# aidalee123/Vision-SR

Measured on NVIDIA B200. Metric: candidate_fits_per_sec, higher is better.
Workload: dtype f64

## Files before the change

vision-sr_b200/csrc/vsr_api.cu:

```cuda
#include <algorithm>
#include <cstdarg>
#include <cstdio>
#include <cstdlib>
#include <cstring>
#include <string>
#include <mutex>
#include <vector>

#include "../../include/vsr.h"
#define VSR_API_TU 1
#include "vsr_launch.h"

namespace {

constexpr int kWidths[] = {0, 1, 2, 3, 4, 5, 6, 7, 8, 12, 16};
constexpr int kNumWidths = sizeof(kWidths) / sizeof(kWidths[0]);

int pick_width(int k) {
  for (int w : kWidths)
    if (w >= k) return w;
  return -1;
}

std::string g_create_error;
// ... 46 lines not shown
  }
};

struct PointSlot {
  const void* X = nullptr;
  const void* y = nullptr;
  int64_t n = 0, ldx = 0;
  int n_vars = 0;
  DevBuf ownX, ownY;
};

}

constexpr int kPoolStreams = 32;
constexpr int kHandleStride = 8;
constexpr int kMaxGroups = 16;
struct StreamPool {
  std::mutex mu;
  std::vector<cudaStream_t> streams;
  int next_base = 0;
};
StreamPool& pool_of(int device) {
  static StreamPool pools[64];
  return pools[device & 63];
}

struct vsr_handle {
  int device = 0;
  int stream_base = 0;
  int num_sms = 148;
  std::string err;
  PointSlot pts[2];
  DevBuf d_insns, d_insn_off, d_imms, d_imm_off, d_k;
  std::vector<int32_t> h_k, h_ninsn, h_nimm, h_nvars;
  std::vector<uint32_t> h_varmask;
  std::vector<cudaStream_t> side_streams;
  cudaEvent_t ev_fork = nullptr;
  std::vector<cudaEvent_t> ev_join;
  int n_programs = 0;
  DevBuf d_lists;
  DevBuf d_partial;
  DevBuf d_stage;
  DevBuf d_queue;
  DevBuf d_handover;
  PinnedBuf h_lists;
  int64_t launches = 0;
  int hook[4] = {0, 0, 0, 0};
  int tile_smem_kb = 200;
  int64_t tile_min_points = 500000;
  int steal_span = 3;
  int latency_k = 0;
  bool queue_by_candidate = false;
  bool handover = true;
  int hold_passes = 500;
  bool profiling = false;
  long long* phase_cycles = nullptr;
  struct Span {
    cudaEvent_t a, b;
    int kind, n;
  };
  std::vector<Span> spans;
  std::vector<cudaEvent_t> event_pool;
};

namespace {

// ... 374 lines not shown
      if (e == cudaSuccess) sp.streams.push_back(s2);
    }
    h->stream_base = sp.next_base;
    sp.next_base = (sp.next_base + kHandleStride) % kPoolStreams;
    for (int i = 0; i < kHandleStride; ++i) h->side_streams.push_back(sp.streams[(h->stream_base + i) % kPoolStreams]);
    for (int i = 0; i < kMaxGroups && e == cudaSuccess; ++i) {
      cudaEvent_t e2;
      e = cudaEventCreateWithFlags(&e2, cudaEventDisableTiming);
      if (e == cudaSuccess) h->ev_join.push_back(e2);
    }
  }
  if (e == cudaSuccess) e = cudaEventCreateWithFlags(&h->ev_fork, cudaEventDisableTiming);
  if (e != cudaSuccess) {
    fail(nullptr, VSR_ECUDA, "allocating the handle's scratch: %s", cudaGetErrorString(e));
    vsr_destroy(h);
    return VSR_ECUDA;
  }
  *out = h;
  return VSR_OK;
}

void vsr_destroy(vsr_handle* h) {
  if (!h) return;
  cudaSetDevice(h->device);
  for (auto& s : h->pts) {
    s.ownX.release();
    s.ownY.release();
  }
  h->d_insns.release();
  h->d_insn_off.release();
  h->d_imms.release();
  h->d_imm_off.release();
  h->d_k.release();
  h->d_lists.release();
  h->d_partial.release();
  h->d_stage.release();
  h->d_queue.release();
  h->d_handover.release();
  h->h_lists.release();
  for (auto e2 : h->ev_join) cudaEventDestroy(e2);
  if (h->ev_fork) cudaEventDestroy(h->ev_fork);
  for (auto& sp : h->spans) {
    if (sp.kind == 0) h->event_pool.push_back(sp.a);
    h->event_pool.push_back(sp.b);
  }
  for (auto e : h->event_pool) cudaEventDestroy(e);
  delete h;
}

const char* vsr_last_error(const vsr_handle* h) { return h ? h->err.c_str() : g_create_error.c_str(); }

int64_t vsr_launch_count(const vsr_handle* h) { return h ? h->launches : 0; }

int vsr_set_phase_buffer(vsr_handle* h, void* dev_i64_nslots_by_8) {
  if (!h) return VSR_EINVAL;
  h->phase_cycles = (long long*)dev_i64_nslots_by_8;
  return VSR_OK;
}

int vsr_set_geometry(vsr_handle* h, int32_t cluster, int32_t threads, int32_t seats, int32_t opt_warps) {
  if (!h) return VSR_EINVAL;
  h->hook[0] = cluster;
  h->hook[1] = threads;
  h->hook[2] = seats;
  h->hook[3] = opt_warps;
  return VSR_OK;
// ... 83 lines not shown
    const int ni = insn_off[c + 1] - insn_off[c];
    const int nm = imm_off[c + 1] - imm_off[c];
    if (ni < 1 || ni > VSR_MAX_INSNS || nm < 0 || nm > VSR_MAX_IMMS || k[c] < 0 || k[c] > VSR_MAX_CONSTS)
      return fail(h, VSR_ELIMIT, "program %d: %d insns, %d literals, %d constants", c, ni, nm, k[c]);
    if (VSR_OP(insns[insn_off[c + 1] - 1]) != VSR_END)
      return fail(h, VSR_EINVAL, "program %d does not end in END", c);
    int sp = 0;
    unsigned var_mask = 0;
    for (int i = insn_off[c]; i < insn_off[c + 1]; ++i) {
      const unsigned op = VSR_OP(insns[i]), src = VSR_SRC(insns[i]), idx = VSR_IDX(insns[i]);
      if (op >= VSR_OP_COUNT) return fail(h, VSR_EINVAL, "program %d: bad opcode %u", c, op);
      if (op == VSR_PUSH && ++sp > VSR_MAX_STACK) return fail(h, VSR_ELIMIT, "program %d: stack too deep", c);
      if (op >= VSR_LOAD && op <= VSR_RPOW && op != VSR_PUSH) {
        if (src == VSR_SRC_STACK) {
          if (--sp < 0) return fail(h, VSR_EINVAL, "program %d: stack underflow", c);
        } else if (src == VSR_SRC_VAR) {
          if (idx >= VSR_MAX_VARS) return fail(h, VSR_EINVAL, "program %d: variable %u", c, idx);
          var_mask |= 1u << idx;
        } else if (src == VSR_SRC_CONST) {
          if ((int)idx >= k[c]) return fail(h, VSR_EINVAL, "program %d: constant %u of %d", c, idx, k[c]);
        } else if (src == VSR_SRC_IMM) {
          if ((int)idx >= nm) return fail(h, VSR_EINVAL, "program %d: literal %u of %d", c, idx, nm);
        } else {
          return fail(h, VSR_EINVAL, "program %d: bad operand source %u", c, src);
        }
      }
    }
    h->h_ninsn[c] = ni;
    h->h_nimm[c] = nm;
    h->h_nvars[c] = __builtin_popcount(var_mask);
    h->h_varmask[c] = var_mask;
  }
  const size_t nins = insn_off[n_programs], nimm = std::max(1, imm_off[n_programs]);
  VSR_CUDA(h, h->d_insns.reserve(nins * sizeof(uint64_t)));
  VSR_CUDA(h, h->d_insn_off.reserve((n_programs + 1) * sizeof(int32_t)));
  VSR_CUDA(h, h->d_imms.reserve(nimm * sizeof(double)));
  VSR_CUDA(h, h->d_imm_off.reserve((n_programs + 1) * sizeof(int32_t)));
  VSR_CUDA(h, h->d_k.reserve(n_programs * sizeof(int32_t)));
  VSR_CUDA(h, cudaMemcpyAsync(h->d_insns.p, insns, nins * sizeof(uint64_t), cudaMemcpyHostToDevice, st));
  VSR_CUDA(h, cudaMemcpyAsync(h->d_insn_off.p, insn_off, (n_programs + 1) * sizeof(int32_t), cudaMemcpyHostToDevice, st));
  if (imm_off[n_programs] > 0)
    VSR_CUDA(h, cudaMemcpyAsync(h->d_imms.p, imms, imm_off[n_programs] * sizeof(double), cudaMemcpyHostToDevice, st));
  VSR_CUDA(h, cudaMemcpyAsync(h->d_imm_off.p, imm_off, (n_programs + 1) * sizeof(int32_t), cudaMemcpyHostToDevice, st));
  VSR_CUDA(h, cudaMemcpyAsync(h->d_k.p, k, n_programs * sizeof(int32_t), cudaMemcpyHostToDevice, st));
  h->n_programs = n_programs;
  return VSR_OK;
}

int vsr_eval(vsr_handle* h, const int32_t* prog_idx, const int32_t* const_row, int32_t n_pairs,
             const double* consts, int32_t kstride, int32_t dtype, double* out_loss,
             double* out_grad, void* stream) {
  int rc = check_ready(h, dtype);
  if (rc) return rc;
  if (!prog_idx || n_pairs <= 0 || !out_loss || kstride < 0 || (!consts && kstride > 0))
    return fail(h, VSR_EINVAL, "bad eval arguments");
  cudaStream_t st = (cudaStream_t)stream;
  VSR_CUDA(h, cudaSetDevice(h->device));
  std::vector<Group> groups(kNumWidths + 1);
  for (int i = 0; i < kNumWidths; ++i) groups[i].K = kWidths[i];
  Group& toowide = groups[kNumWidths];
  for (int p = 0; p < n_pairs; ++p) {
    const int c = prog_idx[p];
    if (c < 0 || c >= h->n_programs) return fail(h, VSR_EINVAL, "pair %d: program %d out of range", p, c);
    const int k = h->h_k[c];
    if (k > kstride) return fail(h, VSR_EINVAL, "pair %d: %d constants > kstride %d", p, k, kstride);
    if ((rc = check_vars(h, c, dtype))) return rc;
    int gi = 0;
    if (out_grad) {
      const int w = pick_width(k);
      if (w < 0) {
        toowide.prog.push_back(p);
        gi = 0;
      } else {
        gi = (int)(std::find(kWidths, kWidths + kNumWidths, w) - kWidths);
      }
    }
    Group& g = groups[gi];
// ... 340 lines not shown
  const bool tma_ok = ((uintptr_t)ps.X % 16 == 0) && ((uintptr_t)ps.y % 16 == 0) && ((ps.ldx * elem) % 16 == 0);
  cudaEvent_t ev_a = nullptr, ev_b = nullptr, ev_c = nullptr;
  if (h->profiling) {
    ev_a = take_event(h);
    ev_b = take_event(h);
    ev_c = take_event(h);
    VSR_CUDA(h, cudaEventRecord(ev_a, st));
  }
  VSR_CUDA(h, h->d_queue.reserve(groups.size() * sizeof(int32_t)));
  VSR_CUDA(h, cudaMemsetAsync(h->d_queue.p, 0, groups.size() * sizeof(int32_t), st));
  std::vector<size_t> ho_off(groups.size() + 1, 0);
  std::vector<int> ho_slot_d(groups.size(), 0);
  if (h->handover) {
    for (size_t gi = 0; gi < groups.size(); ++gi) {
      ho_slot_d[gi] = (vsr::kHandoverHead + vsr::kFitStateDoubles + vsr::fit_workspace_doubles(std::max(1, groups[gi].kmax)) + 1) & ~1;
      ho_off[gi + 1] = ho_off[gi] + 16 + (size_t)vsr::kHandoverSlots * ho_slot_d[gi] * sizeof(double);
    }
    VSR_CUDA(h, h->d_handover.reserve(ho_off.back()));
    VSR_CUDA(h, cudaMemsetAsync(h->d_handover.p, 0, ho_off.back(), st));
  }
  const int hook_cluster = h->hook[0], hook_threads = h->hook[1], hook_seats = h->hook[2], hook_reserved = h->hook[3];

  const size_t n_side = groups.size() > 1 ? groups.size() - 1 : 0;
  if (n_side > h->ev_join.size()) return fail(h, VSR_EINVAL, "%zu launch groups: too many", n_side + 1);
  if (n_side && !h->ev_fork) VSR_CUDA(h, cudaEventCreateWithFlags(&h->ev_fork, cudaEventDisableTiming));
  if (n_side) VSR_CUDA(h, cudaEventRecord(h->ev_fork, st));
  for (size_t gi = 0; gi < groups.size(); ++gi) {
    Group& g = groups[gi];
    const int n = (int)g.prog.size();
    cudaStream_t gs = gi == 0 ? st : h->side_streams[(gi - 1) % h->side_streams.size()];
    if (gi > 0) VSR_CUDA(h, cudaStreamWaitEvent(gs, h->ev_fork, 0));
    vsr::FitArgs a;
    a.pt = table_of(h);
    a.pts = points_of(ps);
    a.run_prog = dl;
    a.run_slot = dl + n_listed;
    a.n_queues = 0;
    for (size_t gj = gi; gj < groups.size() && a.n_queues < vsr::kMaxQueues; ++gj) {
      if (gj > gi && (groups[gj].grad_mode != g.grad_mode || groups[gj].K == 0 || g.K - groups[gj].K > h->steal_span ||
                      gj != gi + (size_t)a.n_queues))
        break;
      a.q_begin[a.n_queues] = g_begin[gj];
      a.q_end[a.n_queues] = g_begin[gj + 1];
      ++a.n_queues;
    }
    for (int q = a.n_queues; q < vsr::kMaxQueues; ++q) a.q_begin[q] = a.q_end[q] = 0;
    a.kstride = kstride;
    a.x0 = x0;
    a.out_consts = out_consts;
    a.out_lastx = out_lastx;
    a.out_loss = out_loss;
    a.out_info = out_info;
    a.O.gtol = opts->gtol;
    a.O.c1 = opts->c1;
    a.O.c2 = opts->c2;
    a.O.xrtol = opts->xrtol;
    a.O.fd_eps = opts->fd_eps;
    a.O.penalty = opts->penalty;
    a.O.loss_scale = opts->loss_scale;
    a.O.stop_time = opts->stop_time;
    a.O.maxiter_per_k = opts->maxiter_per_k;
    a.O.grad_mode = g.grad_mode;
    const int P = points_per_thread(g.K);
    int cap = opts->eval_dtype == VSR_F64 ? fit_threads_cap<double>(g.K) : fit_threads_cap<float>(g.K);
    if (hook_threads > 0) cap = std::min(cap, std::max(32, hook_threads & ~31));
    if (h->latency_k > 0 && g.K >= h->latency_k && hook_threads <= 0) cap = std::min(cap, 320);
// ... 100 lines not shown
```

vision-sr_b200/csrc/vsr_interp.h:

```cpp
#ifndef VSR_INTERP_H_
#define VSR_INTERP_H_

#include "vsr_isa.h"

#if defined(__CUDACC__)
#define VSR_HD __host__ __device__ __forceinline__
#define VSR_MATH __host__ __device__ __noinline__ inline
#else
#include <cmath>
#define VSR_HD inline
#define VSR_MATH inline
#endif

namespace vsr {

#define VSR_M1(Q, name, fd, ff)                 \
  Q double name(double x) { return fd(x); }     \
  Q float name(float x) { return ff(x); }
VSR_M1(VSR_HD, m_sqrt, ::sqrt, ::sqrtf)
VSR_M1(VSR_HD, m_abs, ::fabs, ::fabsf)
VSR_M1(VSR_MATH, m_exp, ::exp, ::expf)
VSR_M1(VSR_MATH, m_log, ::log, ::logf)
VSR_M1(VSR_MATH, m_sin, ::sin, ::sinf)
VSR_M1(VSR_MATH, m_cos, ::cos, ::cosf)
VSR_M1(VSR_MATH, m_tan, ::tan, ::tanf)
VSR_M1(VSR_MATH, m_asin, ::asin, ::asinf)
VSR_M1(VSR_MATH, m_acos, ::acos, ::acosf)
VSR_M1(VSR_MATH, m_atan, ::atan, ::atanf)
VSR_M1(VSR_MATH, m_sinh, ::sinh, ::sinhf)
VSR_M1(VSR_MATH, m_cosh, ::cosh, ::coshf)
VSR_M1(VSR_MATH, m_tanh, ::tanh, ::tanhf)
#undef VSR_M1
VSR_MATH double m_pow(double a, double b) { return ::pow(a, b); }
VSR_MATH float m_pow(float a, float b) { return ::powf(a, b); }
// ... 24 lines not shown
#endif
}
template <typename T>
VSR_HD T m_sign(T x) {
  return x > T(0) ? T(1) : (x < T(0) ? T(-1) : (x == T(0) ? T(0) : x));
}
template <typename T>
VSR_HD T m_powi(T x, int n) {
  T r = T(1);
  T b = x;
  while (n > 0) {
    if (n & 1) r *= b;
    n >>= 1;
    if (n) b *= b;
  }
  return r;
}
template <typename T>
VSR_HD T m_scale(T d, T fp) {
  return d == T(0) ? T(0) : d * fp;
}

template <typename T, int K>
struct Dual {
  T v;
  T d[K > 0 ? K : 1];
};

template <typename T, int K, int P>
struct Stack {
  T s[VSR_MAX_STACK][P][K + 1];
};

template <int OP, typename T, int K>
VSR_HD void unary_apply(Dual<T, K>& x, unsigned am, int n) {
  const T a = x.v;
  const bool live = (K > 0) && am != 0u;
  T f = a, fp = T(1);
  bool guard = false;
  switch (OP) {
    case VSR_NEG:
      f = -a;
      fp = T(-1);
      break;
    case VSR_ABS:
      f = m_abs(a);
      fp = m_sign(a);
      break;
    case VSR_SIGN:
      f = m_sign(a);
      fp = T(0);
      break;
    case VSR_INV:
      f = T(1) / a;
      fp = -f * f;
      break;
    case VSR_SQRT:
      f = m_sqrt(a);
      fp = T(0.5) / f;
      guard = true;
      break;
    case VSR_EXP:
      f = m_exp(a);
      fp = f;
      break;
    case VSR_LOG:
      f = m_log(a);
      fp = T(1) / a;
      break;
    case VSR_SIN:
      if (live) {
        m_sincos(a, &f, &fp);
      } else {
        f = m_sin(a);
      }
      break;
    case VSR_COS:
      if (live) {
        T s;
        m_sincos(a, &s, &f);
        fp = -s;
      } else {
        f = m_cos(a);
      }
      break;
    case VSR_TAN:
      f = m_tan(a);
      fp = T(1) + f * f;
      break;
    case VSR_ASIN:
      f = m_asin(a);
      if (live) fp = T(1) / m_sqrt(T(1) - a * a);
      guard = true;
      break;
    case VSR_ACOS:
      f = m_acos(a);
      if (live) fp = T(-1) / m_sqrt(T(1) - a * a);
      guard = true;
      break;
    case VSR_ATAN:
      f = m_atan(a);
      fp = T(1) / (T(1) + a * a);
      break;
    case VSR_SINH:
      f = m_sinh(a);
      if (live) fp = m_cosh(a);
      break;
    case VSR_COSH:
      f = m_cosh(a);
      if (live) fp = m_sinh(a);
      break;
    case VSR_TANH:
      f = m_tanh(a);
      fp = T(1) - f * f;
      break;
    case VSR_POWI: {
      const int m = n < 0 ? -n : n;
      const T pw = m_powi(a, m - 1);
      const T full = pw * a;
      if (n > 0) {
        f = full;
        fp = T(n) * pw;
      } else {
        f = T(1) / full;
        fp = T(n) * f / a;
      }
      break;
    }
    default:
      break;
  }
  x.v = f;
  if (K > 0) {
    if (guard) {
#pragma unroll
      for (int i = 0; i < K; ++i) x.d[i] = m_scale(x.d[i], fp);
    } else {
#pragma unroll
      for (int i = 0; i < K; ++i) x.d[i] *= fp;
    }
  }
}

#define VSR_H_BINOP(op) ((op) == VSR_LOAD ? 0 : (op)-VSR_ADD + 1)
#define VSR_H_BIN(op, src) (2 + ((VSR_H_BINOP(op)) << 2) + (src))
#define VSR_H_UN(op) (38 + (op)-VSR_NEG)
#define VSR_H_CFOP(op) ((op) == VSR_LOAD ? 0 : (op) == VSR_ADD ? 1 : (op) == VSR_SUB ? 2 : 3)
#define VSR_H_CF(op, j) (55 + VSR_H_CFOP(op) * VSR_MAX_DUAL + (j))
#define VSR_H_END 0
#define VSR_H_PUSH 1
#define VSR_H_COUNT 119
#define VSR_HANDLER(w) ((unsigned)((w)&0xff))

VSR_HD vsr_insn_t predecode(vsr_insn_t w) {
  const unsigned op = VSR_OP(w);
  unsigned h;
  if (op == VSR_END)
    h = VSR_H_END;
  else if (op == VSR_PUSH)
    h = VSR_H_PUSH;
  else if ((op == VSR_LOAD || op == VSR_ADD || op == VSR_SUB || op == VSR_MUL) &&
           (VSR_SRC(w) & 3u) == VSR_SRC_CONST && VSR_IDX(w) < VSR_MAX_DUAL &&
           (op == VSR_LOAD || !((VSR_AMASK(w) >> VSR_IDX(w)) & 1u)))
    h = VSR_H_CF(op, VSR_IDX(w));
  else if (op <= VSR_RPOW)
    h = VSR_H_BIN(op, VSR_SRC(w) & 3u);
  else
    h = VSR_H_UN(op);
  return (w & ~(vsr_insn_t)0xff) | (vsr_insn_t)h;
}

template <int OP, int SRC, typename T, int K, int P, typename XSrc>
VSR_HD void binary_apply(Dual<T, K> (&acc)[P], Stack<T, K, P>& stk, int& sp, unsigned idx,
                         unsigned am, unsigned bm, const double* __restrict__ imm,
                         const T* __restrict__ cst, const XSrc& xs) {
  if (SRC == VSR_SRC_STACK) --sp;
  T ub = T(0);
  if (SRC == VSR_SRC_CONST) ub = cst[idx];
  if (SRC == VSR_SRC_IMM) ub = (T)imm[idx];
  const unsigned lm = am | bm;
#pragma unroll
  for (int p = 0; p < P; ++p) {
    T bv;
    if (SRC == VSR_SRC_STACK)
      bv = stk.s[sp][p][0];
    else if (SRC == VSR_SRC_VAR)
      bv = xs.col(idx, p);
    else
      bv = ub;
    Dual<T, K>& x = acc[p];
#define VSR_TB(i)                                                                   \
  (SRC == VSR_SRC_STACK ? (((bm >> (i)) & 1u) ? stk.s[sp][p][(i) + 1] : T(0))      \
                        : (SRC == VSR_SRC_CONST ? ((i) == (int)idx ? T(1) : T(0)) : T(0)))
    switch (OP) {
      case VSR_LOAD:
        x.v = bv;
#pragma unroll
        for (int i = 0; i < K; ++i) x.d[i] = VSR_TB(i);
        break;
      case VSR_ADD:
        x.v += bv;
        if (SRC == VSR_SRC_STACK) {
#pragma unroll
          for (int i = 0; i < K; ++i)
            if ((bm >> i) & 1u) x.d[i] += stk.s[sp][p][i + 1];
        } else if (SRC == VSR_SRC_CONST) {
#pragma unroll
          for (int i = 0; i < K; ++i) x.d[i] += VSR_TB(i);
        }
        break;
      case VSR_SUB:
        x.v -= bv;
        if (SRC == VSR_SRC_STACK) {
#pragma unroll
          for (int i = 0; i < K; ++i)
            if ((bm >> i) & 1u) x.d[i] -= stk.s[sp][p][i + 1];
        } else if (SRC == VSR_SRC_CONST) {
#pragma unroll
          for (int i = 0; i < K; ++i) x.d[i] -= VSR_TB(i);
        }
        break;
      case VSR_RSUB:
        x.v = bv - x.v;
#pragma unroll
        for (int i = 0; i < K; ++i) x.d[i] = VSR_TB(i) - x.d[i];
        break;
      case VSR_MUL: {
        const T a = x.v;
        x.v = a * bv;
        if (SRC == VSR_SRC_STACK) {
#pragma unroll
          for (int i = 0; i < K; ++i)
            if ((lm >> i) & 1u) x.d[i] = x.d[i] * bv + a * VSR_TB(i);
        } else if (SRC == VSR_SRC_CONST) {
#pragma unroll
          for (int i = 0; i < K; ++i) x.d[i] = x.d[i] * bv + (i == (int)idx ? a : T(0));
        } else {
#pragma unroll
          for (int i = 0; i < K; ++i) x.d[i] *= bv;
        }
        break;
      }
      case VSR_DIV: {
        const T inv = T(1) / bv;
        const T q = x.v / bv;
        if (SRC == VSR_SRC_STACK) {
#pragma unroll
          for (int i = 0; i < K; ++i)
            if ((lm >> i) & 1u) x.d[i] = (x.d[i] - q * VSR_TB(i)) * inv;
        } else if (SRC == VSR_SRC_CONST) {
#pragma unroll
          for (int i = 0; i < K; ++i) x.d[i] = (x.d[i] - (i == (int)idx ? q : T(0))) * inv;
        } else {
#pragma unroll
          for (int i = 0; i < K; ++i) x.d[i] *= inv;
        }
        x.v = q;
        break;
      }
      case VSR_RDIV: {
        const T a = x.v;
        const T inv = T(1) / a;
        const T q = bv / a;
        if (SRC == VSR_SRC_STACK) {
#pragma unroll
          for (int i = 0; i < K; ++i)
            if ((lm >> i) & 1u) x.d[i] = (VSR_TB(i) - q * x.d[i]) * inv;
        } else if (SRC == VSR_SRC_CONST) {
#pragma unroll
          for (int i = 0; i < K; ++i) x.d[i] = ((i == (int)idx ? T(1) : T(0)) - q * x.d[i]) * inv;
        } else {
          const T cf = -q * inv;
#pragma unroll
          for (int i = 0; i < K; ++i) x.d[i] *= cf;
        }
        x.v = q;
        break;
      }
      case VSR_POW: {
        const T a = x.v;
        T lna = T(0);
        const T f = (K == 0) ? m_pow(a, bv) : m_pow_log(a, bv, lna);
        if (K > 0 && lm) {
          const T fa = am ? (a != T(0) ? bv * (f / a) : bv * m_pow(a, bv - T(1))) : T(0);
          T fb = T(0);
          if (bm) fb = (a == T(0) && f == T(0)) ? T(0) : f * lna;
#pragma unroll
          for (int i = 0; i < K; ++i)
            if ((lm >> i) & 1u) x.d[i] = m_scale(x.d[i], fa) + m_scale((T)VSR_TB(i), fb);
        }
        x.v = f;
        break;
      }
      case VSR_RPOW: {
        const T a = x.v;
        T lnb = T(0);
        const T f = (K == 0) ? m_pow(bv, a) : m_pow_log(bv, a, lnb);
        if (K > 0 && lm) {
          T fa = T(0);
          if (am) fa = (bv == T(0) && f == T(0)) ? T(0) : f * lnb;
          const T fb = bm ? (bv != T(0) ? a * (f / bv) : a * m_pow(bv, a - T(1))) : T(0);
#pragma unroll
          for (int i = 0; i < K; ++i)
            if ((lm >> i) & 1u) x.d[i] = m_scale(x.d[i], fa) + m_scale((T)VSR_TB(i), fb);
        }
        x.v = f;
        break;
      }
      default:
        break;
    }
#undef VSR_TB
  }
}

template <int OP, int J, typename T, int K, int P>
VSR_HD void const_fresh_apply(Dual<T, K> (&acc)[P], const T* __restrict__ cst) {
  constexpr int JJ = (K > 0 && J < K) ? J : 0;
  const T c = cst[J];
#pragma unroll
  for (int p = 0; p < P; ++p) {
    Dual<T, K>& x = acc[p];
    const T a = x.v;
    switch (OP) {
      case VSR_LOAD:
        x.v = c;
#pragma unroll
        for (int i = 0; i < K; ++i) x.d[i] = T(0);
        if (K > 0) x.d[JJ] = T(1);
        break;
      case VSR_ADD:
        x.v = a + c;
        if (K > 0) x.d[JJ] = T(1);
        break;
      case VSR_SUB:
        x.v = a - c;
        if (K > 0) x.d[JJ] = T(-1);
        break;
      case VSR_MUL:
        x.v = a * c;
#pragma unroll
        for (int i = 0; i < K; ++i)
          if (i != JJ) x.d[i] *= c;
        if (K > 0) x.d[JJ] = a;
        break;
      default:
        break;
    }
  }
}

template <typename T, int K, int P, typename XSrc>
VSR_HD void eval_points(const vsr_insn_t* __restrict__ prog, const double* __restrict__ imm,
                        const T* __restrict__ cst, const XSrc& xs, Dual<T, K> (&acc)[P],
                        Stack<T, K, P>& stk) {
  int sp = 0;
#pragma unroll
  for (int p = 0; p < P; ++p) {
    acc[p].v = T(0);
#pragma unroll
    for (int i = 0; i < (K > 0 ? K : 1); ++i) acc[p].d[i] = T(0);
  }
  vsr_insn_t w = prog[0];
  for (int pc = 1;; ++pc) {
    const unsigned hid = VSR_HANDLER(w);
    const unsigned idx = VSR_IDX(w);
    const unsigned am = VSR_AMASK(w);
    const unsigned bm = VSR_BMASK(w);
    w = prog[pc];
    switch (hid) {
      case VSR_H_END:
        return;
      case VSR_H_PUSH:
#pragma unroll
        for (int p = 0; p < P; ++p) {
          stk.s[sp][p][0] = acc[p].v;
#pragma unroll
          for (int i = 0; i < K; ++i)
            if ((am >> i) & 1u) stk.s[sp][p][i + 1] = acc[p].d[i];
        }
        ++sp;
        break;
#define VSR_BCASE(OPC)                                                                          \
  case VSR_H_BIN(OPC, VSR_SRC_STACK):                                                           \
    binary_apply<OPC, VSR_SRC_STACK, T, K, P>(acc, stk, sp, idx, am, bm, imm, cst, xs);         \
    break;                                                                                      \
  case VSR_H_BIN(OPC, VSR_SRC_VAR):                                                             \
    binary_apply<OPC, VSR_SRC_VAR, T, K, P>(acc, stk, sp, idx, am, bm, imm, cst, xs);           \
    break;                                                                                      \
  case VSR_H_BIN(OPC, VSR_SRC_CONST):                                                           \
    binary_apply<OPC, VSR_SRC_CONST, T, K, P>(acc, stk, sp, idx, am, bm, imm, cst, xs);         \
    break;                                                                                      \
  case VSR_H_BIN(OPC, VSR_SRC_IMM):                                                             \
    binary_apply<OPC, VSR_SRC_IMM, T, K, P>(acc, stk, sp, idx, am, bm, imm, cst, xs);           \
    break;
        VSR_BCASE(VSR_LOAD)
        VSR_BCASE(VSR_ADD)
        VSR_BCASE(VSR_SUB)
        VSR_BCASE(VSR_RSUB)
        VSR_BCASE(VSR_MUL)
        VSR_BCASE(VSR_DIV)
        VSR_BCASE(VSR_RDIV)
        VSR_BCASE(VSR_POW)
        VSR_BCASE(VSR_RPOW)
#undef VSR_BCASE
#define VSR_CFCASE1(OPC, J)                                              \
  case VSR_H_CF(OPC, J):                                                 \
    if (J < K || K == 0) const_fresh_apply<OPC, J, T, K, P>(acc, cst);   \
    break;
#define VSR_CFCASE(OPC)                                                                          \
  VSR_CFCASE1(OPC, 0) VSR_CFCASE1(OPC, 1) VSR_CFCASE1(OPC, 2) VSR_CFCASE1(OPC, 3)                \
  VSR_CFCASE1(OPC, 4) VSR_CFCASE1(OPC, 5) VSR_CFCASE1(OPC, 6) VSR_CFCASE1(OPC, 7)                \
  VSR_CFCASE1(OPC, 8) VSR_CFCASE1(OPC, 9) VSR_CFCASE1(OPC, 10) VSR_CFCASE1(OPC, 11)              \
  VSR_CFCASE1(OPC, 12) VSR_CFCASE1(OPC, 13) VSR_CFCASE1(OPC, 14) VSR_CFCASE1(OPC, 15)
        VSR_CFCASE(VSR_LOAD)
        VSR_CFCASE(VSR_ADD)
        VSR_CFCASE(VSR_SUB)
        VSR_CFCASE(VSR_MUL)
#undef VSR_CFCASE
#undef VSR_CFCASE1
#define VSR_UCASE(OPC)                                                  \
  case VSR_H_UN(OPC):                                                   \
    _Pragma("unroll") for (int p = 0; p < P; ++p)                       \
        unary_apply<OPC, T, K>(acc[p], am, (int)(int16_t)idx);          \
    break;
        VSR_UCASE(VSR_NEG)
        VSR_UCASE(VSR_ABS)
        VSR_UCASE(VSR_SIGN)
        VSR_UCASE(VSR_INV)
        VSR_UCASE(VSR_SQRT)
        VSR_UCASE(VSR_EXP)
        VSR_UCASE(VSR_LOG)
        VSR_UCASE(VSR_SIN)
        VSR_UCASE(VSR_COS)
        VSR_UCASE(VSR_TAN)
        VSR_UCASE(VSR_ASIN)
        VSR_UCASE(VSR_ACOS)
        VSR_UCASE(VSR_ATAN)
        VSR_UCASE(VSR_SINH)
        VSR_UCASE(VSR_COSH)
        VSR_UCASE(VSR_TANH)
        VSR_UCASE(VSR_POWI)
#undef VSR_UCASE
      default:
#if defined(__CUDA_ARCH__)
        __builtin_unreachable();
#else
        break;
#endif
    }
  }
}

}

#endif
```

vision-sr_b200/csrc/vsr_kernels.cuh:

```cuda
#ifndef VSR_KERNELS_CUH_
#define VSR_KERNELS_CUH_

#include <cooperative_groups.h>
#include <cuda_runtime.h>
#include <stdint.h>

#include "vsr_bfgs.h"
#include "vsr_interp.h"
#include "vsr_isa.h"

namespace vsr {

struct ProgramTable {
  const vsr_insn_t* insns;
  const int32_t* insn_off;
  const double* imms;
  const int32_t* imm_off;
  const int32_t* k;
};

struct Points {
  const void* X;
  const void* y;
  int64_t n;
  int64_t ldx;
};

constexpr int kHandoverSlots = 64;
constexpr unsigned long long kHandoverWaitNs = 300000ull;
constexpr int kHandoverHead = 4;
struct Handover {
  int32_t requests;
  int32_t offers;
  int32_t live;
  int32_t pad;
  double slots[1];
};

constexpr int kMaxSeats = 8;
constexpr int kMaxQueues = 4;

struct FitArgs {
  ProgramTable pt;
  Points pts;
  const int32_t* run_prog;
  const int32_t* run_slot;
  int32_t n_queues;
  int32_t q_begin[kMaxQueues], q_end[kMaxQueues];
  int32_t kstride;
  const double* x0;
  double* out_consts;
  double* out_lastx;
  double* out_loss;
  int32_t* out_info;
  int32_t resident;
  int32_t tma_ok;
  int32_t slice_stride;
  int32_t seats;
  int32_t reserved;
  int32_t seat_d, off_cred, off_ctrl, off_insn;
  int32_t kmax, max_insn, max_imm;
  int32_t n_cols;
  int32_t col_of_var[VSR_MAX_VARS];
  int32_t hold_passes;
  Handover* handover;
  int32_t handover_slot_d;
  int32_t* queue;
  long long* phase_cycles;
  FitOpts O;
};

struct EvalArgs {
  ProgramTable pt;
  Points pts;
  const int32_t* pair_prog;
  const int32_t* pair_row;
// ... 360 lines not shown

struct SeatCtrl {
  int prog;
  int k;
  int n_insn;
  int age;
};

struct SeatBook {
  int slot;
  int prog;
  int k;
  int pad;
  unsigned long long t0;
  double rf;
  long long t_logic, t_seated, n_pass, t_take, t_step, t_pub, ns_seated;
};

template <typename T>
__device__ __forceinline__ void publish_request(const FitArgs& a, int cs, int lane, int prog, int k, bool fresh, int age,
                                                const double* xe, uint32_t ctrl_addr, uint32_t req_bar_addr) {
  int i0 = 0, ni = 0, m0 = 0, nm = 0;
  if (prog >= 0 && fresh) {
    i0 = a.pt.insn_off[prog];
    ni = a.pt.insn_off[prog + 1] - i0;
    m0 = a.pt.imm_off[prog];
    nm = a.pt.imm_off[prog + 1] - m0;
  }
  const uint32_t bytes = 16u + (prog >= 0 ? (uint32_t)k * (uint32_t)sizeof(T) : 0u) +
                         (fresh && prog >= 0 ? (uint32_t)(nm + ni + 1) * 8u : 0u);
  for (int r = lane; r < cs; r += 32) mbar_expect_tx_cluster(mapa_u32(req_bar_addr, r), bytes);
  const uint32_t cst_addr = ctrl_addr + 8u * kSeatCtrlDoubles;
  {
    const int n_items = 2 + (prog >= 0 ? k : 0);
    const int sh = __ffs(cs) - 1;
    for (int idx = lane; idx < (n_items << sh); idx += 32) {
      const int r = idx & (cs - 1), it = idx >> sh;
      const uint32_t bar = mapa_u32(req_bar_addr, r);
      if (it < 2) {
        const uint64_t w = it == 0 ? ((uint64_t)(uint32_t)prog | ((uint64_t)(uint32_t)k << 32))
                                   : ((uint64_t)(uint32_t)ni | ((uint64_t)(uint32_t)age << 32));
        st_async_b64(mapa_u32(ctrl_addr + 8u * it, r), w, bar);
      } else {
        st_async_val(mapa_u32(cst_addr + (uint32_t)(it - 2) * (uint32_t)sizeof(T), r), (T)xe[it - 2], bar);
      }
    }
  }
  if (prog < 0) return;
  if (!fresh) return;
  const uint32_t imm_addr = cst_addr + 8u * kSeatCstDoubles;
  const uint32_t insn_addr = imm_addr + 8u * VSR_MAX_IMMS;
  for (int i = lane; i < nm; i += 32) {
    const double v = a.pt.imms[m0 + i];
    for (int r = 0; r < cs; ++r) st_async_val(mapa_u32(imm_addr + 8u * i, r), v, mapa_u32(req_bar_addr, r));
  }
  for (int i = lane; i <= ni; i += 32) {
    vsr_insn_t w = 0;
    if (i < ni) {
      w = a.pt.insns[i0 + i];
      const unsigned op = VSR_OP(w);
      if (a.resident && op >= VSR_LOAD && op <= VSR_RPOW && op != VSR_PUSH && VSR_SRC(w) == VSR_SRC_VAR)
        w = (w & ~((vsr_insn_t)0xffff << 16)) | ((vsr_insn_t)a.col_of_var[VSR_IDX(w)] << 16);
      w = predecode(w);
    }
    for (int r = 0; r < cs; ++r) st_async_b64(mapa_u32(insn_addr + 8u * i, r), w, mapa_u32(req_bar_addr, r));
  }
}

template <typename T, int K>
__device__ __forceinline__ bool seat_turn(const FitArgs& a, int lane, int cs, FitState& S, double* ws,
                                          const double* cred, SeatBook& book, volatile int* s_qcur, uint64_t* part_bar,
                                          uint32_t ctrl_addr, uint32_t req_bar_addr, const SeatBook* books, int* s_open,
                                          int* s_running) {
  constexpr int W = fit_lanes<K>();
  const bool timing = a.phase_cycles != nullptr && lane == 0;
  long long ta = timing ? clock64() : 0;
  int my_prog = book.prog, my_k = book.k;
  if (my_prog >= 0) {
    const double inv_n = 1.0 / (double)a.pts.n;
    double tot = 0.0;
    if (lane <= K) {
#pragma unroll 8
      for (int r = 0; r < cs; ++r) tot += cred[r * (K + 1) + lane];
    }
    const double f = a.O.loss_scale * (__shfl_sync(0xffffffffu, tot, 0) * inv_n);
    bool bad = !isfinite(f);
    if (a.O.stop_time < 1e8) {
      int late = 0;
      if (lane == 0) {
        const unsigned long long now = global_ns();
        if (book.t0 == 0ull)
          book.t0 = now;
        else if ((double)(now - book.t0) * 1e-9 >= a.O.stop_time)
          late = 1;
      }
      if (__shfl_sync(0xffffffffu, late, 0)) bad = true;
    }
    if (lane >= 1 && lane <= K && lane - 1 < my_k) {
      const double gv = a.O.loss_scale * (2.0 * tot * inv_n);
      ws[my_k + lane - 1] = (bad || !isfinite(gv)) ? 0.0 : gv;
    }
    if (lane == 0) {
      S.rf = bad ? a.O.penalty : f;
      book.n_pass += 1;
      if (timing) book.t_take += clock64() - ta;
    }
    __syncwarp();
  }
  bool fresh = false;
  for (;;) {
    if (my_prog < 0) {
      int r = -1;
      if (a.hold_passes > 0) {
        int hold = 0;
        if (lane == 0) {
          int n_old = 0;
          for (int g2 = 0; g2 < a.seats; ++g2)
            if (&books[g2] != &book && books[g2].prog >= 0 && books[g2].n_pass >= a.hold_passes) ++n_old;
          if (n_old >= 2) {
            if (atomicSub(s_open, 1) > 2)
              hold = 1;
            else
              atomicAdd(s_open, 1);
          }
        }
        if (__shfl_sync(0xffffffffu, hold, 0)) break;
      }
      Handover* const ho = a.handover;
      if (ho != nullptr && lane == 0) atomicAdd(&ho->live, 1);
      for (;;) {
        const int q = *s_qcur;
        if (q >= a.n_queues) break;
        if (lane == 0) r = atomicAdd(a.queue + q, 1) + a.q_begin[q];
// ... 771 lines not shown
```

Baseline: 1558.

## Relabel constants by first use and limit dual-derivative loops to live prefix

Programs are relabeled on the host so constants get dual slots in order of first use, and the kernel maps constants and gradients back through a packed per-program map. The interpreter computes the highest live derivative slot from the activity masks and, when it falls in the lower half, runs only the first K/2 derivative lanes via compile-time index sequences. The aim is to skip multiply-adds on derivative slots that are still zero early in a program. The cost is code-size growth from two unrolled paths per operation, extra branching, and more host preprocessing and device buffers.

```diff
diff --git a/vision-sr_b200/csrc/vsr_api.cu b/vision-sr_b200/csrc/vsr_api.cu
--- a/vision-sr_b200/csrc/vsr_api.cu
+++ b/vision-sr_b200/csrc/vsr_api.cu
@@ -102,6 +102,8 @@
   std::string err;
   PointSlot pts[2];
   DevBuf d_insns, d_insn_off, d_imms, d_imm_off, d_k;
+  DevBuf d_fit_insns, d_const_of;
+  std::vector<uint64_t> h_fit_insns, h_const_of;
   std::vector<int32_t> h_k, h_ninsn, h_nimm, h_nvars;
   std::vector<uint32_t> h_varmask;
   std::vector<cudaStream_t> side_streams;
@@ -542,6 +544,8 @@
   h->d_imms.release();
   h->d_imm_off.release();
   h->d_k.release();
+  h->d_fit_insns.release();
+  h->d_const_of.release();
   h->d_lists.release();
   h->d_partial.release();
   h->d_stage.release();
@@ -691,7 +695,14 @@
     h->h_varmask[c] = var_mask;
   }
   const size_t nins = insn_off[n_programs], nimm = std::max(1, imm_off[n_programs]);
+  h->h_fit_insns.resize(nins);
+  h->h_const_of.resize(n_programs);
+  for (int c = 0; c < n_programs; ++c)
+    h->h_const_of[c] = vsr::relabel_constants(insns + insn_off[c], insn_off[c + 1] - insn_off[c], k[c],
+                                              h->h_fit_insns.data() + insn_off[c]);
   VSR_CUDA(h, h->d_insns.reserve(nins * sizeof(uint64_t)));
+  VSR_CUDA(h, h->d_fit_insns.reserve(nins * sizeof(uint64_t)));
+  VSR_CUDA(h, h->d_const_of.reserve(n_programs * sizeof(uint64_t)));
   VSR_CUDA(h, h->d_insn_off.reserve((n_programs + 1) * sizeof(int32_t)));
   VSR_CUDA(h, h->d_imms.reserve(nimm * sizeof(double)));
   VSR_CUDA(h, h->d_imm_off.reserve((n_programs + 1) * sizeof(int32_t)));
@@ -702,6 +713,10 @@
     VSR_CUDA(h, cudaMemcpyAsync(h->d_imms.p, imms, imm_off[n_programs] * sizeof(double), cudaMemcpyHostToDevice, st));
   VSR_CUDA(h, cudaMemcpyAsync(h->d_imm_off.p, imm_off, (n_programs + 1) * sizeof(int32_t), cudaMemcpyHostToDevice, st));
   VSR_CUDA(h, cudaMemcpyAsync(h->d_k.p, k, n_programs * sizeof(int32_t), cudaMemcpyHostToDevice, st));
+  VSR_CUDA(h, cudaMemcpyAsync(h->d_fit_insns.p, h->h_fit_insns.data(), nins * sizeof(uint64_t),
+                              cudaMemcpyHostToDevice, st));
+  VSR_CUDA(h, cudaMemcpyAsync(h->d_const_of.p, h->h_const_of.data(), n_programs * sizeof(uint64_t),
+                              cudaMemcpyHostToDevice, st));
   h->n_programs = n_programs;
   return VSR_OK;
 }
@@ -1108,6 +1123,8 @@
     if (gi > 0) VSR_CUDA(h, cudaStreamWaitEvent(gs, h->ev_fork, 0));
     vsr::FitArgs a;
     a.pt = table_of(h);
+    a.pt.insns = (const vsr_insn_t*)h->d_fit_insns.p;
+    a.const_of = (const uint64_t*)h->d_const_of.p;
     a.pts = points_of(ps);
     a.run_prog = dl;
     a.run_slot = dl + n_listed;
diff --git a/vision-sr_b200/csrc/vsr_interp.h b/vision-sr_b200/csrc/vsr_interp.h
--- a/vision-sr_b200/csrc/vsr_interp.h
+++ b/vision-sr_b200/csrc/vsr_interp.h
@@ -1,5 +1,8 @@
 #ifndef VSR_INTERP_H_
 #define VSR_INTERP_H_
+
+#include <type_traits>
+#include <utility>
 
 #include "vsr_isa.h"
 
@@ -90,12 +93,31 @@
   T s[VSR_MAX_STACK][P][K + 1];
 };
 
-template <int OP, typename T, int K>
-VSR_HD void unary_apply(Dual<T, K>& x, unsigned am, int n) {
-  const T a = x.v;
-  const bool live = (K > 0) && am != 0u;
-  T f = a, fp = T(1);
-  bool guard = false;
+VSR_HD unsigned mask_len(unsigned m) {
+#if defined(__CUDA_ARCH__)
+  return 32u - (unsigned)__clz((int)m);
+#else
+  return m ? 32u - (unsigned)__builtin_clz(m) : 0u;
+#endif
+}
+
+template <typename F, int... I>
+VSR_HD void each_slot(const F& f, std::integer_sequence<int, I...>) {
+  (f(std::integral_constant<int, I>()), ...);
+}
+
+template <int K, typename F>
+VSR_HD void for_prefix(unsigned hi, const F& f) {
+  if (K >= 4 && hi <= (unsigned)(K / 2))
+    each_slot(f, std::make_integer_sequence<int, K / 2>());
+  else
+    each_slot(f, std::make_integer_sequence<int, K>());
+}
+
+template <int OP, typename T>
+VSR_HD T unary_point(const T a, bool live, int n, T& fp) {
+  T f = a;
+  fp = T(1);
   switch (OP) {
     case VSR_NEG:
       f = -a;
@@ -116,7 +138,6 @@
     case VSR_SQRT:
       f = m_sqrt(a);
       fp = T(0.5) / f;
-      guard = true;
       break;
     case VSR_EXP:
       f = m_exp(a);
@@ -149,12 +170,10 @@
     case VSR_ASIN:
       f = m_asin(a);
       if (live) fp = T(1) / m_sqrt(T(1) - a * a);
-      guard = true;
       break;
     case VSR_ACOS:
       f = m_acos(a);
       if (live) fp = T(-1) / m_sqrt(T(1) - a * a);
-      guard = true;
       break;
     case VSR_ATAN:
       f = m_atan(a);
@@ -188,15 +207,28 @@
     default:
       break;
   }
-  x.v = f;
-  if (K > 0) {
-    if (guard) {
-#pragma unroll
-      for (int i = 0; i < K; ++i) x.d[i] = m_scale(x.d[i], fp);
-    } else {
-#pragma unroll
-      for (int i = 0; i < K; ++i) x.d[i] *= fp;
-    }
+  return f;
+}
+
+template <int OP, typename T, int K, int P>
+VSR_HD void unary_apply(Dual<T, K> (&acc)[P], unsigned am, unsigned hi, int n) {
+  constexpr bool guard = OP == VSR_SQRT || OP == VSR_ASIN || OP == VSR_ACOS;
+  const bool live = (K > 0) && am != 0u;
+  T fp[P];
+#pragma unroll
+  for (int p = 0; p < P; ++p) acc[p].v = unary_point<OP, T>(acc[p].v, live, n, fp[p]);
+  if (guard) {
+    for_prefix<K>(hi, [&](auto ii) {
+      constexpr int i = decltype(ii)::value;
+#pragma unroll
+      for (int p = 0; p < P; ++p) acc[p].d[i] = m_scale(acc[p].d[i], fp[p]);
+    });
+  } else {
+    for_prefix<K>(hi, [&](auto ii) {
+      constexpr int i = decltype(ii)::value;
+#pragma unroll
+      for (int p = 0; p < P; ++p) acc[p].d[i] *= fp[p];
+    });
   }
 }
 
@@ -230,13 +262,17 @@
 
 template <int OP, int SRC, typename T, int K, int P, typename XSrc>
 VSR_HD void binary_apply(Dual<T, K> (&acc)[P], Stack<T, K, P>& stk, int& sp, unsigned idx,
-                         unsigned am, unsigned bm, const double* __restrict__ imm,
+                         unsigned am, unsigned bm, unsigned hi, const double* __restrict__ imm,
                          const T* __restrict__ cst, const XSrc& xs) {
   if (SRC == VSR_SRC_STACK) --sp;
   T ub = T(0);
   if (SRC == VSR_SRC_CONST) ub = cst[idx];
   if (SRC == VSR_SRC_IMM) ub = (T)imm[idx];
   const unsigned lm = am | bm;
+#define VSR_TB(p, i)                                                                \
+  (SRC == VSR_SRC_STACK ? (((bm >> (i)) & 1u) ? stk.s[sp][p][(i) + 1] : T(0))      \
+                        : (SRC == VSR_SRC_CONST ? ((i) == (int)idx ? T(1) : T(0)) : T(0)))
+  T u[P], w[P];
 #pragma unroll
   for (int p = 0; p < P; ++p) {
     T bv;
@@ -247,72 +283,33 @@
     else
       bv = ub;
     Dual<T, K>& x = acc[p];
-#define VSR_TB(i)                                                                   \
-  (SRC == VSR_SRC_STACK ? (((bm >> (i)) & 1u) ? stk.s[sp][p][(i) + 1] : T(0))      \
-                        : (SRC == VSR_SRC_CONST ? ((i) == (int)idx ? T(1) : T(0)) : T(0)))
+    u[p] = w[p] = T(0);
     switch (OP) {
       case VSR_LOAD:
         x.v = bv;
 #pragma unroll
-        for (int i = 0; i < K; ++i) x.d[i] = VSR_TB(i);
+        for (int i = 0; i < K; ++i) x.d[i] = VSR_TB(p, i);
         break;
       case VSR_ADD:
         x.v += bv;
-        if (SRC == VSR_SRC_STACK) {
-#pragma unroll
-          for (int i = 0; i < K; ++i)
-            if ((bm >> i) & 1u) x.d[i] += stk.s[sp][p][i + 1];
-        } else if (SRC == VSR_SRC_CONST) {
-#pragma unroll
-          for (int i = 0; i < K; ++i) x.d[i] += VSR_TB(i);
-        }
         break;
       case VSR_SUB:
         x.v -= bv;
-        if (SRC == VSR_SRC_STACK) {
-#pragma unroll
-          for (int i = 0; i < K; ++i)
-            if ((bm >> i) & 1u) x.d[i] -= stk.s[sp][p][i + 1];
-        } else if (SRC == VSR_SRC_CONST) {
-#pragma unroll
-          for (int i = 0; i < K; ++i) x.d[i] -= VSR_TB(i);
-        }
         break;
       case VSR_RSUB:
         x.v = bv - x.v;
-#pragma unroll
-        for (int i = 0; i < K; ++i) x.d[i] = VSR_TB(i) - x.d[i];
-        break;
-      case VSR_MUL: {
-        const T a = x.v;
-        x.v = a * bv;
-        if (SRC == VSR_SRC_STACK) {
-#pragma unroll
-          for (int i = 0; i < K; ++i)
-            if ((lm >> i) & 1u) x.d[i] = x.d[i] * bv + a * VSR_TB(i);
-        } else if (SRC == VSR_SRC_CONST) {
-#pragma unroll
-          for (int i = 0; i < K; ++i) x.d[i] = x.d[i] * bv + (i == (int)idx ? a : T(0));
-        } else {
-#pragma unroll
-          for (int i = 0; i < K; ++i) x.d[i] *= bv;
-        }
-        break;
-      }
+        break;
+      case VSR_MUL:
+        u[p] = x.v;
+        w[p] = bv;
+        x.v = u[p] * bv;
+        break;
       case VSR_DIV: {
         const T inv = T(1) / bv;
         const T q = x.v / bv;
-        if (SRC == VSR_SRC_STACK) {
-#pragma unroll
-          for (int i = 0; i < K; ++i)
-            if ((lm >> i) & 1u) x.d[i] = (x.d[i] - q * VSR_TB(i)) * inv;
-        } else if (SRC == VSR_SRC_CONST) {
-#pragma unroll
-          for (int i = 0; i < K; ++i) x.d[i] = (x.d[i] - (i == (int)idx ? q : T(0))) * inv;
-        } else {
-#pragma unroll
-          for (int i = 0; i < K; ++i) x.d[i] *= inv;
-        }
+        u[p] = q;
+        w[p] = inv;
+        if (SRC == VSR_SRC_VAR || SRC == VSR_SRC_IMM) u[p] = inv;
         x.v = q;
         break;
       }
@@ -320,18 +317,9 @@
         const T a = x.v;
         const T inv = T(1) / a;
         const T q = bv / a;
-        if (SRC == VSR_SRC_STACK) {
-#pragma unroll
-          for (int i = 0; i < K; ++i)
-            if ((lm >> i) & 1u) x.d[i] = (VSR_TB(i) - q * x.d[i]) * inv;
-        } else if (SRC == VSR_SRC_CONST) {
-#pragma unroll
-          for (int i = 0; i < K; ++i) x.d[i] = ((i == (int)idx ? T(1) : T(0)) - q * x.d[i]) * inv;
-        } else {
-          const T cf = -q * inv;
-#pragma unroll
-          for (int i = 0; i < K; ++i) x.d[i] *= cf;
-        }
+        u[p] = q;
+        w[p] = inv;
+        if (SRC == VSR_SRC_VAR || SRC == VSR_SRC_IMM) u[p] = -q * inv;
         x.v = q;
         break;
       }
@@ -340,12 +328,8 @@
         T lna = T(0);
         const T f = (K == 0) ? m_pow(a, bv) : m_pow_log(a, bv, lna);
         if (K > 0 && lm) {
-          const T fa = am ? (a != T(0) ? bv * (f / a) : bv * m_pow(a, bv - T(1))) : T(0);
-          T fb = T(0);
-          if (bm) fb = (a == T(0) && f == T(0)) ? T(0) : f * lna;
-#pragma unroll
-          for (int i = 0; i < K; ++i)
-            if ((lm >> i) & 1u) x.d[i] = m_scale(x.d[i], fa) + m_scale((T)VSR_TB(i), fb);
+          u[p] = am ? (a != T(0) ? bv * (f / a) : bv * m_pow(a, bv - T(1))) : T(0);
+          if (bm) w[p] = (a == T(0) && f == T(0)) ? T(0) : f * lna;
         }
         x.v = f;
         break;
@@ -355,12 +339,8 @@
         T lnb = T(0);
         const T f = (K == 0) ? m_pow(bv, a) : m_pow_log(bv, a, lnb);
         if (K > 0 && lm) {
-          T fa = T(0);
-          if (am) fa = (bv == T(0) && f == T(0)) ? T(0) : f * lnb;
-          const T fb = bm ? (bv != T(0) ? a * (f / bv) : a * m_pow(bv, a - T(1))) : T(0);
-#pragma unroll
-          for (int i = 0; i < K; ++i)
-            if ((lm >> i) & 1u) x.d[i] = m_scale(x.d[i], fa) + m_scale((T)VSR_TB(i), fb);
+          if (am) u[p] = (bv == T(0) && f == T(0)) ? T(0) : f * lnb;
+          w[p] = bm ? (bv != T(0) ? a * (f / bv) : a * m_pow(bv, a - T(1))) : T(0);
         }
         x.v = f;
         break;
@@ -368,18 +348,79 @@
       default:
         break;
     }
+  }
+  if (OP == VSR_LOAD) return;
+  for_prefix<K>(hi, [&](auto ii) {
+    constexpr int i = decltype(ii)::value;
+#pragma unroll
+    for (int p = 0; p < P; ++p) {
+      T& d = acc[p].d[i];
+      switch (OP) {
+        case VSR_ADD:
+          if (SRC == VSR_SRC_STACK) {
+            if ((bm >> i) & 1u) d += stk.s[sp][p][i + 1];
+          } else if (SRC == VSR_SRC_CONST) {
+            d += VSR_TB(p, i);
+          }
+          break;
+        case VSR_SUB:
+          if (SRC == VSR_SRC_STACK) {
+            if ((bm >> i) & 1u) d -= stk.s[sp][p][i + 1];
+          } else if (SRC == VSR_SRC_CONST) {
+            d -= VSR_TB(p, i);
+          }
+          break;
+        case VSR_RSUB:
+          d = VSR_TB(p, i) - d;
+          break;
+        case VSR_MUL:
+          if (SRC == VSR_SRC_STACK) {
+            if ((lm >> i) & 1u) d = d * w[p] + u[p] * VSR_TB(p, i);
+          } else if (SRC == VSR_SRC_CONST) {
+            d = d * w[p] + (i == (int)idx ? u[p] : T(0));
+          } else {
+            d *= w[p];
+          }
+          break;
+        case VSR_DIV:
+          if (SRC == VSR_SRC_STACK) {
+            if ((lm >> i) & 1u) d = (d - u[p] * VSR_TB(p, i)) * w[p];
+          } else if (SRC == VSR_SRC_CONST) {
+            d = (d - (i == (int)idx ? u[p] : T(0))) * w[p];
+          } else {
+            d *= u[p];
+          }
+          break;
+        case VSR_RDIV:
+          if (SRC == VSR_SRC_STACK) {
+            if ((lm >> i) & 1u) d = (VSR_TB(p, i) - u[p] * d) * w[p];
+          } else if (SRC == VSR_SRC_CONST) {
+            d = ((i == (int)idx ? T(1) : T(0)) - u[p] * d) * w[p];
+          } else {
+            d *= u[p];
+          }
+          break;
+        case VSR_POW:
+        case VSR_RPOW:
+          if ((lm >> i) & 1u) d = m_scale(d, u[p]) + m_scale((T)VSR_TB(p, i), w[p]);
+          break;
+        default:
+          break;
+      }
+    }
+  });
 #undef VSR_TB
-  }
 }
 
 template <int OP, int J, typename T, int K, int P>
-VSR_HD void const_fresh_apply(Dual<T, K> (&acc)[P], const T* __restrict__ cst) {
+VSR_HD void const_fresh_apply(Dual<T, K> (&acc)[P], unsigned hi, const T* __restrict__ cst) {
   constexpr int JJ = (K > 0 && J < K) ? J : 0;
   const T c = cst[J];
+  T a[P];
 #pragma unroll
   for (int p = 0; p < P; ++p) {
     Dual<T, K>& x = acc[p];
-    const T a = x.v;
+    a[p] = x.v;
     switch (OP) {
       case VSR_LOAD:
         x.v = c;
@@ -388,23 +429,30 @@
         if (K > 0) x.d[JJ] = T(1);
         break;
       case VSR_ADD:
-        x.v = a + c;
+        x.v = a[p] + c;
         if (K > 0) x.d[JJ] = T(1);
         break;
       case VSR_SUB:
-        x.v = a - c;
+        x.v = a[p] - c;
         if (K > 0) x.d[JJ] = T(-1);
         break;
       case VSR_MUL:
-        x.v = a * c;
-#pragma unroll
-        for (int i = 0; i < K; ++i)
-          if (i != JJ) x.d[i] *= c;
-        if (K > 0) x.d[JJ] = a;
+        x.v = a[p] * c;
         break;
       default:
         break;
     }
+  }
+  if (OP == VSR_MUL && K > 0) {
+    for_prefix<K>(hi, [&](auto ii) {
+      constexpr int i = decltype(ii)::value;
+      if (i != JJ) {
+#pragma unroll
+        for (int p = 0; p < P; ++p) acc[p].d[i] *= c;
+      }
+    });
+#pragma unroll
+    for (int p = 0; p < P; ++p) acc[p].d[JJ] = a[p];
   }
 }
 
@@ -425,32 +473,35 @@
     const unsigned idx = VSR_IDX(w);
     const unsigned am = VSR_AMASK(w);
     const unsigned bm = VSR_BMASK(w);
+    const unsigned hi = mask_len(am | bm);
     w = prog[pc];
     switch (hid) {
       case VSR_H_END:
         return;
       case VSR_H_PUSH:
 #pragma unroll
-        for (int p = 0; p < P; ++p) {
-          stk.s[sp][p][0] = acc[p].v;
-#pragma unroll
-          for (int i = 0; i < K; ++i)
-            if ((am >> i) & 1u) stk.s[sp][p][i + 1] = acc[p].d[i];
-        }
+        for (int p = 0; p < P; ++p) stk.s[sp][p][0] = acc[p].v;
+        for_prefix<K>(hi, [&](auto ii) {
+          constexpr int i = decltype(ii)::value;
+          if ((am >> i) & 1u) {
+#pragma unroll
+            for (int p = 0; p < P; ++p) stk.s[sp][p][i + 1] = acc[p].d[i];
+          }
+        });
         ++sp;
         break;
 #define VSR_BCASE(OPC)                                                                          \
   case VSR_H_BIN(OPC, VSR_SRC_STACK):                                                           \
-    binary_apply<OPC, VSR_SRC_STACK, T, K, P>(acc, stk, sp, idx, am, bm, imm, cst, xs);         \
+    binary_apply<OPC, VSR_SRC_STACK, T, K, P>(acc, stk, sp, idx, am, bm, hi, imm, cst, xs);         \
     break;                                                                                      \
   case VSR_H_BIN(OPC, VSR_SRC_VAR):                                                             \
-    binary_apply<OPC, VSR_SRC_VAR, T, K, P>(acc, stk, sp, idx, am, bm, imm, cst, xs);           \
+    binary_apply<OPC, VSR_SRC_VAR, T, K, P>(acc, stk, sp, idx, am, bm, hi, imm, cst, xs);           \
     break;                                                                                      \
   case VSR_H_BIN(OPC, VSR_SRC_CONST):                                                           \
-    binary_apply<OPC, VSR_SRC_CONST, T, K, P>(acc, stk, sp, idx, am, bm, imm, cst, xs);         \
+    binary_apply<OPC, VSR_SRC_CONST, T, K, P>(acc, stk, sp, idx, am, bm, hi, imm, cst, xs);         \
     break;                                                                                      \
   case VSR_H_BIN(OPC, VSR_SRC_IMM):                                                             \
-    binary_apply<OPC, VSR_SRC_IMM, T, K, P>(acc, stk, sp, idx, am, bm, imm, cst, xs);           \
+    binary_apply<OPC, VSR_SRC_IMM, T, K, P>(acc, stk, sp, idx, am, bm, hi, imm, cst, xs);           \
     break;
         VSR_BCASE(VSR_LOAD)
         VSR_BCASE(VSR_ADD)
@@ -464,7 +515,7 @@
 #undef VSR_BCASE
 #define VSR_CFCASE1(OPC, J)                                              \
   case VSR_H_CF(OPC, J):                                                 \
-    if (J < K || K == 0) const_fresh_apply<OPC, J, T, K, P>(acc, cst);   \
+    if (J < K || K == 0) const_fresh_apply<OPC, J, T, K, P>(acc, hi, cst);   \
     break;
 #define VSR_CFCASE(OPC)                                                                          \
   VSR_CFCASE1(OPC, 0) VSR_CFCASE1(OPC, 1) VSR_CFCASE1(OPC, 2) VSR_CFCASE1(OPC, 3)                \
@@ -479,8 +530,7 @@
 #undef VSR_CFCASE1
 #define VSR_UCASE(OPC)                                                  \
   case VSR_H_UN(OPC):                                                   \
-    _Pragma("unroll") for (int p = 0; p < P; ++p)                       \
-        unary_apply<OPC, T, K>(acc[p], am, (int)(int16_t)idx);          \
+    unary_apply<OPC, T, K, P>(acc, am, hi, (int)(int16_t)idx);          \
     break;
         VSR_UCASE(VSR_NEG)
         VSR_UCASE(VSR_ABS)
diff --git a/vision-sr_b200/csrc/vsr_kernels.cuh b/vision-sr_b200/csrc/vsr_kernels.cuh
--- a/vision-sr_b200/csrc/vsr_kernels.cuh
+++ b/vision-sr_b200/csrc/vsr_kernels.cuh
@@ -8,6 +8,7 @@
 #include "vsr_bfgs.h"
 #include "vsr_interp.h"
 #include "vsr_isa.h"
+#include "vsr_relabel.h"
 
 namespace vsr {
 
@@ -42,6 +43,7 @@
 
 struct FitArgs {
   ProgramTable pt;
+  const uint64_t* const_of;
   Points pts;
   const int32_t* run_prog;
   const int32_t* run_slot;
@@ -468,6 +470,7 @@
   for (int r = lane; r < cs; r += 32) mbar_expect_tx_cluster(mapa_u32(req_bar_addr, r), bytes);
   const uint32_t cst_addr = ctrl_addr + 8u * kSeatCtrlDoubles;
   {
+    const uint64_t const_of = prog >= 0 ? a.const_of[prog] : kIdentityConstOf;
     const int n_items = 2 + (prog >= 0 ? k : 0);
     const int sh = __ffs(cs) - 1;
     for (int idx = lane; idx < (n_items << sh); idx += 32) {
@@ -478,7 +481,8 @@
                                    : ((uint64_t)(uint32_t)ni | ((uint64_t)(uint32_t)age << 32));
         st_async_b64(mapa_u32(ctrl_addr + 8u * it, r), w, bar);
       } else {
-        st_async_val(mapa_u32(cst_addr + (uint32_t)(it - 2) * (uint32_t)sizeof(T), r), (T)xe[it - 2], bar);
+        st_async_val(mapa_u32(cst_addr + (uint32_t)(it - 2) * (uint32_t)sizeof(T), r),
+                     (T)xe[const_of_slot(const_of, it - 2)], bar);
       }
     }
   }
@@ -513,6 +517,7 @@
   long long ta = timing ? clock64() : 0;
   int my_prog = book.prog, my_k = book.k;
   if (my_prog >= 0) {
+    const uint64_t const_of = __ldg(a.const_of + my_prog);
     const double inv_n = 1.0 / (double)a.pts.n;
     double tot = 0.0;
     if (lane <= K) {
@@ -534,7 +539,7 @@
     }
     if (lane >= 1 && lane <= K && lane - 1 < my_k) {
       const double gv = a.O.loss_scale * (2.0 * tot * inv_n);
-      ws[my_k + lane - 1] = (bad || !isfinite(gv)) ? 0.0 : gv;
+      ws[my_k + const_of_slot(const_of, lane - 1)] = (bad || !isfinite(gv)) ? 0.0 : gv;
     }
     if (lane == 0) {
       S.rf = bad ? a.O.penalty : f;
diff --git a/vision-sr_b200/csrc/vsr_relabel.h b/vision-sr_b200/csrc/vsr_relabel.h
--- /dev/null
+++ b/vision-sr_b200/csrc/vsr_relabel.h
@@ -0,0 +1,64 @@
+#ifndef VSR_RELABEL_H_
+#define VSR_RELABEL_H_
+
+#include <stdint.h>
+
+#include "vsr_isa.h"
+
+#if defined(__CUDACC__)
+#define VSR_RELABEL_HD __host__ __device__ __forceinline__
+#else
+#define VSR_RELABEL_HD inline
+#endif
+
+namespace vsr {
+
+VSR_RELABEL_HD unsigned const_of_slot(uint64_t const_of, int s) {
+  return s < VSR_MAX_DUAL ? (unsigned)((const_of >> (4 * s)) & 0xfu) : (unsigned)s;
+}
+constexpr uint64_t kIdentityConstOf = 0xfedcba9876543210ull;
+
+inline uint64_t relabel_constants(const vsr_insn_t* in, int n, int k, vsr_insn_t* out) {
+  if (k > VSR_MAX_DUAL) {
+    for (int i = 0; i < n; ++i) out[i] = in[i];
+    return kIdentityConstOf;
+  }
+  int slot_of[VSR_MAX_DUAL], const_of[VSR_MAX_DUAL], used = 0;
+  for (int j = 0; j < VSR_MAX_DUAL; ++j) slot_of[j] = -1;
+  for (int i = 0; i < n; ++i) {
+    const unsigned op = VSR_OP(in[i]), idx = VSR_IDX(in[i]);
+    if (op >= VSR_LOAD && op <= VSR_RPOW && op != VSR_PUSH && VSR_SRC(in[i]) == VSR_SRC_CONST &&
+        (int)idx < k && slot_of[idx] < 0) {
+      slot_of[idx] = used;
+      const_of[used++] = (int)idx;
+    }
+  }
+  for (int j = 0; j < k; ++j)
+    if (slot_of[j] < 0) {
+      slot_of[j] = used;
+      const_of[used++] = j;
+    }
+  for (int j = k; j < VSR_MAX_DUAL; ++j) slot_of[j] = j;
+  uint64_t map = kIdentityConstOf;
+  for (int s = 0; s < k; ++s)
+    map = (map & ~(0xfull << (4 * s))) | ((uint64_t)const_of[s] << (4 * s));
+  auto remap = [&](unsigned m) {
+    unsigned r = 0;
+    for (int j = 0; j < VSR_MAX_DUAL; ++j)
+      if ((m >> j) & 1u) r |= 1u << slot_of[j];
+    return r;
+  };
+  for (int i = 0; i < n; ++i) {
+    const vsr_insn_t w = in[i];
+    const unsigned op = VSR_OP(w);
+    unsigned idx = VSR_IDX(w);
+    if (op >= VSR_LOAD && op <= VSR_RPOW && op != VSR_PUSH && VSR_SRC(w) == VSR_SRC_CONST && (int)idx < k)
+      idx = (unsigned)slot_of[idx];
+    out[i] = VSR_INSN(op, VSR_SRC(w), idx, remap(VSR_AMASK(w)), remap(VSR_BMASK(w)));
+  }
+  return map;
+}
+
+}
+
+#endif
```

Measured after the change: 1500 (median of 6 runs). 3.7% lower.
